# ultralytics/yolov3

Measured on NVIDIA H100. Metric: images/sec @640 bs32 YOLOv3, higher is better.
Workload: dtype bf16

## Files before the change

### include/yolov3_b200.h

```cpp
#ifndef YOLOV3_B200_H
#define YOLOV3_B200_H

#include <stddef.h>
#include <stdint.h>

#ifdef __cplusplus
extern "C" {
#endif

#define Y3_OK 0
#define Y3_ERR_BAD_ARG (-1)
#define Y3_ERR_CUDA (-2)
#define Y3_ERR_UNSUPPORTED (-3)

#define Y3_ACT_NONE 0
#define Y3_ACT_SILU 1

typedef void* y3_stream_t;

int y3_version(void);
int y3_last_error(char* buf, size_t n);
int y3_device_check(void);
int64_t y3_abi_sizeof(int32_t which);
int y3_set_pdl(int32_t on);

typedef struct y3_conv_desc {
  int32_t n, h, w;
  int32_t c_in, c_out;
  int32_t ksize, stride;
  int32_t act;
  const void* in;
  int32_t in_ld, in_coff;
  const void* weight;
  const float* bias;
  void* out;
  int32_t out_ld, out_coff;
  const void* res;
  int32_t res_ld, res_coff;
  int32_t upsample;
  float* out_f32;
  int32_t out_f32_ld;
  int32_t* err;
  int32_t weight_layout;
  int32_t in_fmt;
  int32_t out_fmt;
  const float* dq;
  float res_scale;
  float out_inv_scale;
} y3_conv_desc;
#define Y3_FMT_BF16 0
#define Y3_FMT_E4M3 1
int y3_conv_bn_act_fwd(const y3_conv_desc* d, y3_stream_t stream);
int y3_conv_dgrad_s2(const y3_conv_desc* d, y3_stream_t stream);
#define Y3_W_TAPS 0
#define Y3_W_XPAIR 1
int y3_conv_weight_layout(const y3_conv_desc* d);
typedef struct y3_conv_plan_info {
  int32_t block_n, block_k, halo, resident_weights, xpair;
  int32_t m_tiles, n_tiles, k_blocks, grid;
} y3_conv_plan_info;
int y3_conv_plan(const y3_conv_desc* d, y3_conv_plan_info* out);
int y3_conv_cout_pad(int32_t c_out);

#define Y3_IN_F32 0
#define Y3_IN_U8 1
typedef struct y3_first_desc {
  const void* in;
  int32_t in_dtype;
  float in_div;
  int32_t n, h, w;
  const float* weight;
  const float* bias;
  int32_t c_out;
  void* out;
  int32_t out_ld, out_coff;
} y3_first_desc;
int y3_conv_first_fwd(const y3_first_desc* d, y3_stream_t stream);

typedef struct y3_pool_desc {
  const void* in;
  int32_t in_ld, in_coff;
  void* out;
  int32_t out_ld, out_coff;
  int32_t n, h, w, c;
  int32_t ho, wo;
  int32_t k, stride, off, oob_zero;
  int32_t fmt;
} y3_pool_desc;
int y3_maxpool_fwd(const y3_pool_desc* d, y3_stream_t stream);
int y3_maxpool_train_fwd(const y3_pool_desc* d, uint8_t* idx, y3_stream_t stream);
int y3_maxpool_bwd(const y3_pool_desc* d, const uint8_t* idx, int32_t accumulate, y3_stream_t stream);

int y3_amax_nhwc(const void* x, int32_t fmt, int32_t ld, int32_t coff, int32_t n, int32_t h, int32_t w, int32_t c,
                 float* amax, y3_stream_t stream);

int y3_nchw_to_padded_nhwc(const float* src, int32_t n, int32_t c, int32_t h, int32_t w, void* dst, int32_t dst_ld,
                           int32_t dst_coff, y3_stream_t stream);
int y3_padded_nhwc_to_nchw(const void* src, int32_t src_ld, int32_t src_coff, int32_t n, int32_t c, int32_t h,
                           int32_t w, float* dst, y3_stream_t stream);

#define Y3_MAX_LEVELS 5
#define Y3_MAX_ANCHORS 6
typedef struct y3_detect_level {
  const float* raw;
  const float* head;
  int32_t head_ld;
  float* raw_out;
  int32_t ny, nx;
  float stride;
  float anchor_w[Y3_MAX_ANCHORS];
  float anchor_h[Y3_MAX_ANCHORS];
} y3_detect_level;
// ... 257 lines not shown
```

### yolov3_b200/_lib.py

```python
from __future__ import annotations

import ctypes as C
from pathlib import Path

_LIB_PATH = Path(__file__).resolve().parent / "libyolov3_b200.so"
_lib = None


class Y3Error(RuntimeError):
    pass


class ConvDesc(C.Structure):

    _fields_ = [
        ("n", C.c_int32), ("h", C.c_int32), ("w", C.c_int32),
        ("c_in", C.c_int32), ("c_out", C.c_int32),
        ("ksize", C.c_int32), ("stride", C.c_int32),
        ("act", C.c_int32),
        ("in_", C.c_void_p), ("in_ld", C.c_int32), ("in_coff", C.c_int32),
        ("weight", C.c_void_p),
        ("bias", C.c_void_p),
        ("out", C.c_void_p), ("out_ld", C.c_int32), ("out_coff", C.c_int32),
        ("res", C.c_void_p), ("res_ld", C.c_int32), ("res_coff", C.c_int32),
        ("upsample", C.c_int32),
        ("out_f32", C.c_void_p), ("out_f32_ld", C.c_int32),
        ("err", C.c_void_p),
        ("weight_layout", C.c_int32),
        ("in_fmt", C.c_int32), ("out_fmt", C.c_int32),
        ("dq", C.c_void_p), ("res_scale", C.c_float), ("out_inv_scale", C.c_float),
    ]


class ConvPlanInfo(C.Structure):

    _fields_ = [(k, C.c_int32) for k in ("block_n", "block_k", "halo", "resident_weights", "xpair", "m_tiles", "n_tiles",
                                         "k_blocks", "grid")]


W_TAPS, W_XPAIR = 0, 1
FMT_BF16, FMT_E4M3 = 0, 1
MAX_LEVELS, MAX_ANCHORS = 5, 6


class DetectLevel(C.Structure):

    _fields_ = [("raw", C.c_void_p), ("head", C.c_void_p), ("head_ld", C.c_int32), ("raw_out", C.c_void_p),
                ("ny", C.c_int32), ("nx", C.c_int32), ("stride", C.c_float),
                ("anchor_w", C.c_float * MAX_ANCHORS), ("anchor_h", C.c_float * MAX_ANCHORS)]


class FirstDesc(C.Structure):

    _fields_ = [("in_", C.c_void_p), ("in_dtype", C.c_int32), ("in_div", C.c_float),
                ("n", C.c_int32), ("h", C.c_int32), ("w", C.c_int32),
                ("weight", C.c_void_p), ("bias", C.c_void_p), ("c_out", C.c_int32),
                ("out", C.c_void_p), ("out_ld", C.c_int32), ("out_coff", C.c_int32)]


class PoolDesc(C.Structure):

    _fields_ = [("in_", C.c_void_p), ("in_ld", C.c_int32), ("in_coff", C.c_int32),
                ("out", C.c_void_p), ("out_ld", C.c_int32), ("out_coff", C.c_int32),
                ("n", C.c_int32), ("h", C.c_int32), ("w", C.c_int32), ("c", C.c_int32),
                ("ho", C.c_int32), ("wo", C.c_int32),
                ("k", C.c_int32), ("stride", C.c_int32), ("off", C.c_int32), ("oob_zero", C.c_int32),
                ("fmt", C.c_int32)]


class DecodeDesc(C.Structure):

    _fields_ = [("levels", DetectLevel * MAX_LEVELS), ("nl", C.c_int32), ("bs", C.c_int32), ("na", C.c_int32),
                ("no", C.c_int32), ("z", C.c_void_p)]


OP_CONV_FIRST, OP_CONV, OP_MAXPOOL, OP_DECODE, OP_AMAX = 1, 2, 3, 4, 5
IN_F32, IN_U8 = 0, 1


class AmaxDesc(C.Structure):

    _fields_ = [("x", C.c_void_p), ("fmt", C.c_int32), ("ld", C.c_int32), ("coff", C.c_int32),
                ("n", C.c_int32), ("h", C.c_int32), ("w", C.c_int32), ("c", C.c_int32), ("amax", C.c_void_p)]


class Op(C.Structure):

    _fields_ = [("kind", C.c_int32), ("conv", ConvDesc), ("first", FirstDesc), ("pool", PoolDesc),
                ("decode", DecodeDesc), ("amax", AmaxDesc)]

# ... 244 lines not shown
```

### yolov3_b200/csrc/y3_conv_tc.cu

```cuda
#include <cuda_bf16.h>

#include <type_traits>

#include "y3_common.cuh"
#include "y3_internal.h"

namespace y3 {

namespace {

constexpr int kBlockM = 128;
constexpr int kThreads = 320;
constexpr int kProducerWarp = 8;
constexpr int kStoreWarp = 9;
constexpr int kSmemBudget = 221 * 1024;

template <int BLOCK_N, int BLOCK_K, bool HALO, int STAGE_ES = 2, bool STAGE_DQ = false>
struct Cfg {
  static constexpr uint32_t kARows = HALO ? kBlockM + 2 : kBlockM;
  static constexpr uint32_t kATxBytes = kARows * BLOCK_K * 2;
  static constexpr uint32_t kABytes = (kATxBytes + 1023u) / 1024u * 1024u;
  static constexpr uint32_t kTaps = HALO ? 3 : 1;
  static constexpr uint32_t kBBytes = BLOCK_N * BLOCK_K * 2;
  static constexpr uint32_t kStageBytes = kABytes + kTaps * kBBytes;
  static constexpr int kMaxStages = 8;
  static constexpr uint32_t kBarBytes = 256;
  static constexpr uint32_t kRowBytes = BLOCK_N * (STAGE_ES > 0 ? STAGE_ES : 2);
  static constexpr uint32_t kTileBytes = kBlockM * kRowBytes;
  static constexpr uint32_t kBoxBytes = kRowBytes < 128 ? kRowBytes : 128;
  static constexpr uint32_t kBoxes = kRowBytes / kBoxBytes;
  static constexpr int kBufs = STAGE_ES == 0 ? 0 : (kTileBytes > 32 * 1024 ? 1 : 2);
  static constexpr bool kSBias = BLOCK_N == 256 && kBufs > 0;
  static constexpr uint32_t kBiasBytes = kSBias ? BLOCK_N * 4 * (STAGE_DQ ? 2 : 1) : 0;
  static constexpr uint32_t kTileReserve = 1024 - kBarBytes + kBufs * (kTileBytes + kBiasBytes);
  __host__ __device__ static constexpr int ring_stages(uint32_t reserve) {
    const int s = int(kSmemBudget - reserve) / int(kStageBytes);
    return s > kMaxStages ? kMaxStages : s;
  }
  __host__ __device__ static constexpr uint32_t bres_bytes(int steps) { return (uint32_t(steps) * kBBytes + 1023u) / 1024u * 1024u; }
  __host__ __device__ static constexpr int bres_stages(int steps, uint32_t reserve) {
    const int s = (int(kSmemBudget - reserve) - int(bres_bytes(steps))) / int(kABytes);
    return s > kMaxStages ? kMaxStages : s;
  }
  static constexpr uint32_t kSwizzleBytes = BLOCK_K * 2;
  static constexpr uint32_t kSbo = 8 * kSwizzleBytes;
  __host__ __device__ static constexpr uint32_t bar_offset(int stages, bool bres, int b_steps) {
    return uint32_t(stages) * kABytes + (bres ? bres_bytes(b_steps) : uint32_t(stages) * kTaps * kBBytes);
  }
  __host__ __device__ static constexpr uint32_t smem_end(int stages, bool bres, int b_steps, uint32_t reserve) {
    return bar_offset(stages, bres, b_steps) + kBarBytes + reserve;
  }
  static constexpr size_t kSmemBytes = size_t(kSmemBudget) + 1024  + kBarBytes;
  static_assert(ring_stages(kTileReserve) >= 2, "pipeline needs at least two stages");
  static_assert(!HALO || BLOCK_K >= 32, "halo reuse: rows of 64 or 128 bytes");
};

__device__ __forceinline__ float bias_act(float a, float b, bool silu) {
  if (!silu) return a + b;
  const float h = fmaf(a, 0.5f, b);
  float t;
  asm("tanh.approx.f32 %0, %1;" : "=f"(t) : "f"(h));
  return fmaf(h, t, h);
}

__device__ __forceinline__ float bias_act_dq(float a, float s, float b, bool silu) {
  const float h = fmaf(a, s, b);
  if (!silu) return h;
  float t;
  asm("tanh.approx.f32 %0, %1;" : "=f"(t) : "f"(h));
  return fmaf(h, t, h);
}

__device__ __forceinline__ uint32_t fast_div(uint32_t n, uint32_t mul, uint32_t shr) {
  const uint32_t t = __umulhi(n, mul);
  return (t + ((n - t) >> (shr ? 1 : 0))) >> (shr ? shr - 1 : 0);
}

struct RowOut {
  __nv_bfloat16* out;
  float* f32;
  const __nv_bfloat16* res;
};

template <int ES, typename T>
__device__ __forceinline__ T* elem_ptr(T* p, long long off) {
  if (ES == 2) return p + off;
  return reinterpret_cast<T*>(reinterpret_cast<uintptr_t>(p) + off * ES);
}

template <int ES = 2>
__device__ __forceinline__ RowOut row_out(const ConvTcArgs& p, int mt, int n0, int m) {
  RowOut o{nullptr, nullptr, nullptr};
  bool valid;
  int img, oy, ox;
  if (p.mode == 0) {
    const int row = mt * kBlockM + m;
    const int plane = p.hp * p.wp;
    img = static_cast<int>(fast_div(static_cast<uint32_t>(row), p.plane_mul, p.plane_shr));
    const int rem = row - img * plane;
    const int yp = static_cast<int>(fast_div(static_cast<uint32_t>(rem), p.wp_mul, p.wp_shr)), xp = rem - yp * p.wp;
    valid = row < p.rows_total && yp >= 1 && yp <= p.hp - 2 && xp >= 1 && xp <= p.wp - 2;
    oy = yp - 1;
    ox = xp - 1;
  } else {
    const int per_img = p.tiles_w * p.tiles_h;
    img = mt / per_img;
    const int t = mt - img * per_img;
    const int ty = m / p.tw, tx = m - ty * p.tw;
    oy = (t / p.tiles_w) * p.th + ty;
    ox = (t % p.tiles_w) * p.tw + tx;
    valid = ty < p.th && oy < p.ho && ox < p.wo;
  }
  if (!valid) return o;
  const int oh = p.mode == 0 ? p.hp - 2 : p.ho;
  const int ow = p.mode == 0 ? p.wp - 2 : p.wo;
  long long conv_row = (static_cast<long long>(img) * (oh + 2) + oy + 1) * (ow + 2) + ox + 1;
  if (p.phase)
    conv_row = (static_cast<long long>(img) * (2 * oh + 2) + 2 * oy + p.ph_a + 1) * (2 * ow + 2) + 2 * ox + p.ph_b + 1;
  if (p.res) o.res = elem_ptr<ES>(p.res, conv_row * p.res_ld + p.res_coff + n0);
  if (p.out_f32) {
    o.f32 = p.out_f32 + ((static_cast<long long>(img) * oh + oy) * ow + ox) * p.out_f32_ld + n0;
  } else if (p.upsample) {
    const long long r00 = (static_cast<long long>(img) * (2 * oh + 2) + 2 * oy + 1) * (2 * ow + 2) + 2 * ox + 1;
    o.out = elem_ptr<ES>(p.out, r00 * p.out_ld + p.out_coff + n0);
  } else {
    o.out = elem_ptr<ES>(p.out, conv_row * p.out_ld + p.out_coff + n0);
  }
  return o;
}

template <int BLOCK_N, int BLOCK_K, bool HALO, int IN_FMT = Y3_FMT_BF16, int OUT_FMT = Y3_FMT_BF16>
__global__ void __launch_bounds__(kThreads, 1)
conv_tc_kernel(const __grid_constant__ CUtensorMap map_a, const __grid_constant__ CUtensorMap map_b,
               const __grid_constant__ CUtensorMap map_out, const __grid_constant__ CUtensorMap map_res, const ConvTcArgs p) {
  constexpr bool kInE4m3 = IN_FMT == Y3_FMT_E4M3, kOutE4m3 = OUT_FMT == Y3_FMT_E4M3;
  using C = Cfg<BLOCK_N, BLOCK_K, HALO, kOutE4m3 ? 1 : (kInE4m3 ? 0 : 2), kInE4m3 && kOutE4m3>;
  constexpr int kOes = kOutE4m3 ? 1 : 2;
  constexpr int kKch = kInE4m3 ? 2 * BLOCK_K : BLOCK_K;
  using Mma = std::conditional_t<kInE4m3, WgmmaE4m3<BLOCK_N>, Wgmma<BLOCK_N>>;
  const int STAGES = p.stages;
  const bool bres = p.bres != 0;
  constexpr uint32_t kBStage = C::kTaps * C::kBBytes;
  const int b_steps = p.taps * p.kblocks;

  extern __shared__ uint8_t smem_raw[];
  const uint32_t raw_addr = smem_u32(smem_raw);
  uint8_t* smem = smem_raw + ((1024u - (raw_addr & 1023u)) & 1023u);
  uint8_t* smem_a = smem;
  uint8_t* smem_b = smem + STAGES * C::kABytes;
  uint64_t* full_bar = reinterpret_cast<uint64_t*>(smem_b + (bres ? C::bres_bytes(b_steps) : uint32_t(STAGES) * kBStage));
  uint64_t* empty_bar = full_bar + C::kMaxStages;
  uint64_t* bres_bar = empty_bar + C::kMaxStages;
  uint64_t* staged_bar = bres_bar + 1;
  uint64_t* done_bar = bres_bar + 3;
  uint8_t* otile = reinterpret_cast<uint8_t*>(full_bar) + 1024;
  const bool tile_out = C::kBufs > 0 && p.tile_tma != 0;
  constexpr int kBufs = C::kBufs > 0 ? C::kBufs : 1;

  const int warp = threadIdx.x >> 5;
  const int lane = threadIdx.x & 31;

  if (threadIdx.x == 0) {
    tma_prefetch_desc(&map_a);
    tma_prefetch_desc(&map_b);
    if (tile_out) {
      tma_prefetch_desc(&map_out);
      if (p.res) tma_prefetch_desc(&map_res);
    }
    for (int i = 0; i < STAGES; ++i) {
      mbar_init(&full_bar[i], 1);
      mbar_init(&empty_bar[i], 8);
    }
    mbar_init(bres_bar, 1);
    for (int b = 0; b < 2; ++b) {
      mbar_init(&staged_bar[b], 1);
      mbar_init(&done_bar[b], 8);
    }
    fence_mbar_init();
  }
  __syncthreads();
  pdl_wait();
  pdl_trigger();

  const int total_tiles = p.m_tiles * p.n_tiles;
  const int k_iters = HALO ? 3 * p.kblocks : p.taps * p.kblocks;

  if (warp == kProducerWarp) {
    uint32_t stage = 0, phase = 0;
    if (bres && int(blockIdx.x) < total_tiles && elect_one()) {
      mbar_expect_tx(bres_bar, uint32_t(b_steps) * C::kBBytes);
      for (int st = 0; st < b_steps; ++st) {
        const int kb = st / p.taps, tap = st - kb * p.taps;
        tma_load_2d(smem_b + st * C::kBBytes, &map_b, bres_bar, (p.custom_taps ? p.tap_wcol[tap] : tap) * p.cin + kb * kKch, 0);
      }
    }
    __syncwarp();
    const int n_tiles = p.n_tiles, wp = p.wp, cin = p.cin, a_coff = p.a_coff, a_ld = p.a_ld;
    const int taps_it = HALO ? 3 : p.taps;
    const bool xpair = p.xpair != 0, nine = p.taps == 9, custom = p.custom_taps != 0;
    const int taps_w = xpair ? 2 : 3;
    const uint32_t stage_tx = p.a_tx_bytes + (bres ? 0u : kBStage);
    auto run = [&](auto mode_tag) {
      constexpr int MODE = decltype(mode_tag)::value;
      for (int tile = blockIdx.x; tile < total_tiles; tile += gridDim.x) {
        const int nt = tile % n_tiles;
        const int mt = tile / n_tiles;
        const int n0 = nt * BLOCK_N;
        int row0 = 0, img = 0, oh0 = 0, ow0 = 0;
        if (MODE == 0) {
          row0 = mt * kBlockM;
        } else {
          const int per_img = p.tiles_w * p.tiles_h;
          img = mt / per_img;
          const int t = mt - img * per_img;
          oh0 = (t / p.tiles_w) * p.th;
          ow0 = (t % p.tiles_w) * p.tw;
        }
        int kb = 0, tap = 0, r = 0, s = 0;
        for (int it = 0; it < k_iters; ++it) {
          mbar_wait(&empty_bar[stage], phase ^ 1u, p.err, 1);
          if (elect_one()) {
            uint8_t* a_dst = smem_a + stage * C::kABytes;
            uint8_t* b_dst = smem_b + stage * kBStage;
            const int kcol = kb * kKch;
            const int shift = HALO ? (tap - 1) * wp - 1 : (custom ? p.tap_shift[tap] : (nine ? (r - 1) * wp + (s - 1) : 0));
            const int c0 = xpair ? a_coff : (s & 1) * a_ld + a_coff + kcol;
            const int c1 = xpair ? s : (s >> 1);
            const int bcol = (HALO ? tap * 3 : (custom ? p.tap_wcol[tap] : tap)) * cin + kcol;
            mbar_expect_tx(&full_bar[stage], stage_tx);
            if (MODE == 0)
              tma_load_2d(a_dst, &map_a, &full_bar[stage], a_coff + kcol, row0 + shift);
            else
              tma_load_5d(a_dst, &map_a, &full_bar[stage], c0, ow0 + c1, r & 1, oh0 + (r >> 1), img);
            if (!bres) {
#pragma unroll
              for (uint32_t t = 0; t < C::kTaps; ++t)
                tma_load_2d(b_dst + t * C::kBBytes, &map_b, &full_bar[stage], bcol + int(t) * cin, n0);
            }
          }
          __syncwarp();
          if (++stage == uint32_t(STAGES)) {
            stage = 0;
            phase ^= 1u;
          }
          if (++s == taps_w) {
            s = 0;
            ++r;
          }
          if (++tap == taps_it) {
            tap = 0;
            r = 0;
            s = 0;
            ++kb;
          }
        }
      }
    };
    if (p.mode == 0)
      run(std::integral_constant<int, 0>{});
    else
      run(std::integral_constant<int, 1>{});
  } else if (warp == kStoreWarp) {
    if (tile_out) {
      if (lane != 0) return;
      const uint32_t res_tx = uint32_t(p.mode == 0 ? kBlockM : p.tw * p.th) * C::kRowBytes;
      constexpr int kBoxCh = C::kBoxBytes / kOes;
      auto move = [&](int tile, int b, bool load) {
        const int mt = tile / p.n_tiles, n0 = (tile % p.n_tiles) * BLOCK_N;
        int c1 = mt * kBlockM, c2 = 0, c3 = 0;
        if (p.mode != 0) {
          const int per_img = p.tiles_w * p.tiles_h;
          c3 = mt / per_img;
          const int t = mt - c3 * per_img;
          c1 = (t % p.tiles_w) * p.tw;
          c2 = (t / p.tiles_w) * p.th;
        }
#pragma unroll
        for (uint32_t k = 0; k < C::kBoxes; ++k) {
          uint8_t* s = otile + b * C::kTileBytes + k * kBlockM * C::kBoxBytes;
          const int c0 = (load ? p.res_coff : p.out_coff) + n0 + int(k) * kBoxCh;
          if (load) {
            if (p.mode == 0) tma_load_2d(s, &map_res, &staged_bar[b], c0, c1);
            else tma_load_4d(s, &map_res, &staged_bar[b], c0, c1, c2, c3);
          } else {
            if (p.mode == 0) tma_store_2d(&map_out, s, c0, c1);
            else tma_store_4d(&map_out, s, c0, c1, c2, c3);
          }
        }
      };
      auto stage = [&](int tile, int b) {
        const int n0 = (tile % p.n_tiles) * BLOCK_N;
        const uint32_t bias_tx = C::kSBias ? uint32_t(min(BLOCK_N, p.cout - n0)) * 4u : 0u;
        const uint32_t tx = (p.res ? res_tx : 0u) + bias_tx * (kInE4m3 ? 2u : 1u);
        if (tx == 0) {
          mbar_arrive(&staged_bar[b]);
          return;
        }
        mbar_expect_tx(&staged_bar[b], tx);
        if (p.res) move(tile, b, true);
        if constexpr (C::kSBias) {
          uint8_t* sb = otile + C::kBufs * C::kTileBytes + b * C::kBiasBytes;
          bulk_load(sb, p.bias + n0, bias_tx, &staged_bar[b]);
          if (kInE4m3) bulk_load(sb + BLOCK_N * 4, p.dq + n0, bias_tx, &staged_bar[b]);
        }
      };
      const int step = int(gridDim.x);
#pragma unroll
      for (int i = 0; i < kBufs; ++i)
        if (int(blockIdx.x) + i * step < total_tiles) stage(blockIdx.x + i * step, i);
      for (int tile = blockIdx.x, i = 0; tile < total_tiles; tile += step, ++i) {
        const int b = i % kBufs;
        mbar_wait(&done_bar[b], uint32_t(i / kBufs) & 1u, p.err, 9);
        move(tile, b, false);
        bulk_commit_group();
        if (tile + kBufs * step < total_tiles) {
          bulk_wait_read_all();
          stage(tile + kBufs * step, b);
        }
      }
      bulk_wait_all();
    }
  } else {
    const int wg = warp >> 2;
    const int m0 = wg * 64 + (warp & 3) * 16 + (lane >> 2);
    const int cq = 2 * (lane & 3);
    constexpr uint32_t kDescHi = wgmma_desc_hi(C::kSbo, C::kSwizzleBytes);
    const uint32_t a_base = smem_u32(smem_a) + uint32_t(wg) * 64u * C::kSwizzleBytes;
    const uint32_t b_base = smem_u32(smem_b);
    uint32_t stage = 0, phase = 0;
    if (bres && int(blockIdx.x) < total_tiles) mbar_wait(bres_bar, 0, p.err, 6);
    for (int tile = blockIdx.x; tile < total_tiles; tile += gridDim.x) {
      float acc[BLOCK_N / 2];
      uint32_t prev = 0;
      for (int it = 0; it < k_iters; ++it) {
        mbar_wait(&full_bar[stage], phase, p.err, 3);
        const uint32_t a_st = a_base + stage * C::kABytes;
        const uint32_t b_st = b_base + (bres ? uint32_t(it) : stage) * kBStage;
        wgmma_fence();
#pragma unroll
        for (uint32_t t = 0; t < C::kTaps; ++t) {
#pragma unroll
          for (int k = 0; k < BLOCK_K / 16; ++k) {
            const uint64_t adesc = wgmma_desc(kDescHi, a_st + t * C::kSwizzleBytes + k * 32);
            const uint64_t bdesc = wgmma_desc(kDescHi, b_st + t * C::kBBytes + k * 32);
            Mma::template mma<0, 0>(acc, adesc, bdesc, (it != 0 || t != 0 || k != 0) ? 1u : 0u);
          }
        }
        wgmma_commit();
        wgmma_wait<1>();
        if (it > 0 && lane == 0) mbar_arrive(&empty_bar[prev]);
        prev = stage;
        if (++stage == uint32_t(STAGES)) {
          stage = 0;
          phase ^= 1u;
        }
      }
      wgmma_wait<0>();
      wgmma_fence_regs(acc);
      if (lane == 0) mbar_arrive(&empty_bar[prev]);

      const bool silu = p.act == Y3_ACT_SILU;
      const float bscale = silu ? 0.5f : 1.0f;
      if (tile_out) {
        const int ti = (tile - int(blockIdx.x)) / int(gridDim.x);
        const int b = ti % kBufs;
        mbar_wait(&staged_bar[b], uint32_t(ti / kBufs) & 1u, p.err, 10);
        const int n0 = (tile % p.n_tiles) * BLOCK_N;
        const bool has_res = p.res != nullptr;
        const uint32_t sw = ((uint32_t(m0) * C::kBoxBytes >> 7) & (C::kBoxBytes / 16 - 1)) << 4;
        const uint32_t row_s = ((smem_u32(otile) + uint32_t(m0) * C::kBoxBytes + cq * kOes) ^ sw) + b * C::kTileBytes;
        const uint32_t bias_s = smem_u32(otile) + C::kBufs * C::kTileBytes + b * C::kBiasBytes + cq * 4;
        bool valid[2] = {true, true};
        if (p.mode == 0) {
#pragma unroll
          for (int h = 0; h < 2; ++h) {
            const int row = (tile / p.n_tiles) * kBlockM + m0 + 8 * h;
            const int img = static_cast<int>(fast_div(static_cast<uint32_t>(row), p.plane_mul, p.plane_shr));
            const int rem = row - img * (p.hp * p.wp);
            const int yp = static_cast<int>(fast_div(static_cast<uint32_t>(rem), p.wp_mul, p.wp_shr)), xp = rem - yp * p.wp;
            valid[h] = yp >= 1 && yp <= p.hp - 2 && xp >= 1 && xp <= p.wp - 2;
          }
        }
#pragma unroll
        for (int j = 0; j < BLOCK_N / 8; ++j) {
          const int c = 8 * j + cq;
          float2 bv, qv;
          if constexpr (C::kSBias) {
            bv = lds_f32x2(bias_s + 32 * j);
            qv = kInE4m3 ? lds_f32x2(bias_s + 4 * BLOCK_N + 32 * j) : bv;
          } else {
            const bool in = n0 + c < p.cout;
            bv = in ? __ldg(reinterpret_cast<const float2*>(p.bias + n0 + c)) : make_float2(0.f, 0.f);
            qv = bv;
            if (kInE4m3) qv = in ? __ldg(reinterpret_cast<const float2*>(p.dq + n0 + c)) : make_float2(0.f, 0.f);
          }
          const uint32_t xb = uint32_t(8 * j * kOes);
          const uint32_t region = xb / C::kBoxBytes * (kBlockM * C::kBoxBytes), xin = xb % C::kBoxBytes;
#pragma unroll
          for (int h = 0; h < 2; ++h) {
            const uint32_t pp = (row_s ^ xin) + region + 8 * h * C::kBoxBytes;
            float x0, x1;
            if (kInE4m3) {
              x0 = bias_act_dq(acc[4 * j + 2 * h], bscale * qv.x, bscale * bv.x, silu);
              x1 = bias_act_dq(acc[4 * j + 2 * h + 1], bscale * qv.y, bscale * bv.y, silu);
            } else {
              x0 = bias_act(acc[4 * j + 2 * h], bscale * bv.x, silu);
              x1 = bias_act(acc[4 * j + 2 * h + 1], bscale * bv.y, silu);
            }
            if constexpr (kOutE4m3) {
              if (has_res) {
                const float2 f = unpack_e4m3x2(lds16(pp));
                x0 = fmaf(p.res_scale, f.x, x0);
// ... 28 lines not shown
            uint32_t r[kChunk];
#pragma unroll
            for (int jj = 0; jj < kChunk; ++jj) {
              const int c = 8 * (j0 + jj) + cq;
              const bool in = p.out_f32 || n0 + c < p.cout;
              b[jj] = in ? __ldg(reinterpret_cast<const float2*>(p.bias + n0 + c)) : make_float2(0.f, 0.f);
              if (kInE4m3) q[jj] = in ? __ldg(reinterpret_cast<const float2*>(p.dq + n0 + c)) : make_float2(0.f, 0.f);
              if (kOutE4m3)
                r[jj] = (in && ro.res) ? __ldcg(reinterpret_cast<const unsigned short*>(elem_ptr<1>(ro.res, c))) : 0u;
              else
                r[jj] = (in && ro.res) ? __ldcg(reinterpret_cast<const unsigned int*>(ro.res + c)) : 0u;
            }
#pragma unroll
            for (int jj = 0; jj < kChunk; ++jj) {
              const int c = 8 * (j0 + jj) + cq;
              if (!p.out_f32 && n0 + c >= p.cout) continue;
              float x0, x1;
              if (kInE4m3) {
                x0 = bias_act_dq(acc[4 * (j0 + jj) + 2 * h], bscale * q[jj].x, bscale * b[jj].x, silu);
                x1 = bias_act_dq(acc[4 * (j0 + jj) + 2 * h + 1], bscale * q[jj].y, bscale * b[jj].y, silu);
              } else {
                x0 = bias_act(acc[4 * (j0 + jj) + 2 * h], bscale * b[jj].x, silu);
                x1 = bias_act(acc[4 * (j0 + jj) + 2 * h + 1], bscale * b[jj].y, silu);
              }
              if (ro.f32) {
                *reinterpret_cast<float2*>(ro.f32 + c) = make_float2(x0, x1);
              } else if (kOutE4m3) {
                if (ro.res) {
                  const float2 f = unpack_e4m3x2(static_cast<uint16_t>(r[jj]));
                  x0 = fmaf(p.res_scale, f.x, x0);
                  x1 = fmaf(p.res_scale, f.y, x1);
                }
                const uint16_t v = pack_e4m3x2(x0 * p.out_inv_scale, x1 * p.out_inv_scale);
                for (int rep = 0; rep < reps; ++rep)
                  *reinterpret_cast<uint16_t*>(elem_ptr<1>(ro.out, (rep >> 1) * up_row_stride + (rep & 1) * p.out_ld + c)) = v;
              } else {
                if (ro.res) {
                  const float2 f = unpack_bf16x2(r[jj]);
                  x0 += f.x;
                  x1 += f.y;
                }
                const uint32_t v = pack_bf16x2(x0, x1);
                for (int rep = 0; rep < reps; ++rep)
                  *reinterpret_cast<uint32_t*>(ro.out + (rep >> 1) * up_row_stride + (rep & 1) * p.out_ld + c) = v;
              }
            }
          }
        }
      }
    }
  }
}

template <int BLOCK_N, int BLOCK_K, bool HALO = false, int IN_FMT = Y3_FMT_BF16, int OUT_FMT = Y3_FMT_BF16>
int launch_cfg(const ConvTcPlan& plan, cudaStream_t stream) {
  constexpr bool kInE4m3 = IN_FMT == Y3_FMT_E4M3, kOutE4m3 = OUT_FMT == Y3_FMT_E4M3;
  using C = Cfg<BLOCK_N, BLOCK_K, HALO, kOutE4m3 ? 1 : (kInE4m3 ? 0 : 2), kInE4m3 && kOutE4m3>;
  auto kern = conv_tc_kernel<BLOCK_N, BLOCK_K, HALO, IN_FMT, OUT_FMT>;
  static bool attr_set = false;
  if (!attr_set) {
    Y3_CHECK_CUDA(cudaFuncSetAttribute(kern, cudaFuncAttributeMaxDynamicSharedMemorySize, int(C::kSmemBytes)));
    attr_set = true;
  }
  ConvTcArgs args = plan.args;
  const uint32_t reserve = (C::kBufs > 0 && args.tile_tma != 0) ? C::kTileReserve : 0u;
  const int b_steps = args.taps * args.kblocks;
  args.bres = plan.bres;
  args.stages = plan.bres ? C::bres_stages(b_steps, reserve) : C::ring_stages(reserve);
  if (args.bres && args.stages < 3) {
    args.bres = 0;
    args.stages = C::ring_stages(reserve);
  }
  if (args.stages < 2 || args.stages > C::kMaxStages ||
      C::smem_end(args.stages, args.bres != 0, b_steps, reserve) + 1024u > C::kSmemBytes)
    return set_error(Y3_ERR_BAD_ARG, "conv_tc: %d ring stages (resident weights %d, output tiles %u bytes) do not fit %zu bytes of shared memory (N=%d K=%d)",
                     args.stages, args.bres, reserve, C::kSmemBytes, BLOCK_N, BLOCK_K);
  Y3_CHECK_CUDA(launch_pdl(kern, dim3(plan.grid), dim3(kThreads), C::kSmemBytes, stream, plan.map_a, plan.map_b,
                           plan.map_out, plan.map_res, args));
  return Y3_OK;
}

int pick_block_n(int cout) { return cout <= 32 ? 32 : (cout <= 64 ? 64 : (cout <= 128 ? 128 : 256)); }

template <int IN_FMT, int OUT_FMT>
int launch_fmt(const ConvTcPlan& plan, cudaStream_t stream) {
#define Y3_DISPATCH_K(BN)                                                        \
  switch (plan.block_k) {                                                        \
    case 64: return launch_cfg<BN, 64, false, IN_FMT, OUT_FMT>(plan, stream);    \
    case 32: return launch_cfg<BN, 32, false, IN_FMT, OUT_FMT>(plan, stream);    \
    case 16: return launch_cfg<BN, 16, false, IN_FMT, OUT_FMT>(plan, stream);    \
  }                                                                              \
  break;
  constexpr bool kHalo = !(IN_FMT == Y3_FMT_E4M3 && OUT_FMT == Y3_FMT_BF16);
  if (plan.halo) {
    if constexpr (kHalo) {
      if (plan.block_k == 64) {
        if (plan.block_n == 128) return launch_cfg<128, 64, true, IN_FMT, OUT_FMT>(plan, stream);
        if (plan.block_n == 64) return launch_cfg<64, 64, true, IN_FMT, OUT_FMT>(plan, stream);
        if (plan.block_n == 32) return launch_cfg<32, 64, true, IN_FMT, OUT_FMT>(plan, stream);
      } else if (plan.block_k == 32) {
        if (plan.block_n == 64) return launch_cfg<64, 32, true, IN_FMT, OUT_FMT>(plan, stream);
        if (plan.block_n == 32) return launch_cfg<32, 32, true, IN_FMT, OUT_FMT>(plan, stream);
      }
    }
    return set_error(Y3_ERR_BAD_ARG, "conv_tc: no halo kernel for tile N=%d K=%d (formats %d -> %d)", plan.block_n,
                     plan.block_k, IN_FMT, OUT_FMT);
  }
  switch (plan.block_n) {
    case 32: Y3_DISPATCH_K(32)
    case 64: Y3_DISPATCH_K(64)
    case 128: Y3_DISPATCH_K(128)
    case 256: Y3_DISPATCH_K(256)
  }
#undef Y3_DISPATCH_K
  return set_error(Y3_ERR_BAD_ARG, "conv_tc: no kernel for tile N=%d K=%d", plan.block_n, plan.block_k);
}

}

int conv_tc_launch(const ConvTcPlan& plan, cudaStream_t stream) {
  if (plan.in_fmt == Y3_FMT_BF16 && plan.out_fmt == Y3_FMT_BF16) return launch_fmt<Y3_FMT_BF16, Y3_FMT_BF16>(plan, stream);
  if (plan.in_fmt == Y3_FMT_BF16 && plan.out_fmt == Y3_FMT_E4M3) return launch_fmt<Y3_FMT_BF16, Y3_FMT_E4M3>(plan, stream);
  if (plan.in_fmt == Y3_FMT_E4M3 && plan.out_fmt == Y3_FMT_E4M3) return launch_fmt<Y3_FMT_E4M3, Y3_FMT_E4M3>(plan, stream);
  if (plan.in_fmt == Y3_FMT_E4M3 && plan.out_fmt == Y3_FMT_BF16) return launch_fmt<Y3_FMT_E4M3, Y3_FMT_BF16>(plan, stream);
  return set_error(Y3_ERR_BAD_ARG, "conv_tc: formats %d -> %d", plan.in_fmt, plan.out_fmt);
}

static void fast_div_for(uint32_t d, uint32_t* mul, uint32_t* shr) {
  if (d <= 1) {
    *mul = 0;
    *shr = 0;
    return;
  }
  uint32_t l = 0;
  while ((1ull << l) < d) ++l;
  *mul = static_cast<uint32_t>(((1ull << 32) * ((1ull << l) - d)) / d + 1);
  *shr = l;
}

static bool conv_prefers_xpair(const y3_conv_desc& d) {
  return d.in_fmt == Y3_FMT_BF16 && d.ksize == 3 && d.stride == 2 && (d.c_in == 32 || d.c_in == 16) && d.in_ld == d.c_in && d.in_coff == 0;
}

int conv_tc_prepare(const y3_conv_desc& d, ConvTcPlan* plan, bool select_only, const ConvTcExtra* extra) {
  Y3_REQUIRE(d.n > 0 && d.h > 0 && d.w > 0, "conv: empty shape");
  Y3_REQUIRE((d.ksize == 1 && d.stride == 1) || (d.ksize == 3 && (d.stride == 1 || d.stride == 2)),
// ... 49 lines not shown
  const int kch = bk * 2 / es;
  const int cout_pad = (d.c_out + bn - 1) / bn * bn;
  const int taps = extra ? extra->ntaps : (xpair ? 6 : d.ksize * d.ksize);
  const int hp = d.h + 2, wp = d.w + 2;
  if (extra) Y3_REQUIRE(d.stride == 1 && !xpair && !head && !d.upsample && extra->ntaps >= 1 && extra->ntaps <= 4, "conv: bad custom tap list");

  ConvTcArgs& a = plan->args;
  a = ConvTcArgs{};
  plan->in_fmt = d.in_fmt;
  plan->out_fmt = out8 ? Y3_FMT_E4M3 : Y3_FMT_BF16;
  plan->block_n = bn;
  plan->block_k = bk;
  a.taps = taps;
  a.kblocks = gemm_cin / kch;
  a.cin = gemm_cin;
  a.xpair = xpair ? 1 : 0;
  a.a_coff = d.in_coff;
  a.a_ld = d.in_ld;
  a.n_tiles = cout_pad / bn;
  a.bias = d.bias;
  a.cout = d.c_out;
  a.act = d.act;
  a.out = static_cast<__nv_bfloat16*>(d.out);
  a.out_ld = d.out_ld;
  a.out_coff = d.out_coff;
  a.upsample = d.upsample;
  a.res = static_cast<const __nv_bfloat16*>(d.res);
  a.res_ld = d.res_ld;
  a.res_coff = d.res_coff;
  a.out_f32 = d.out_f32;
  a.out_f32_ld = d.out_f32_ld;
  a.err = d.err;
  a.dq = in8 ? d.dq : nullptr;
  a.res_scale = d.res_scale;
  a.out_inv_scale = d.out_inv_scale;
  if (head) {
    a.out = nullptr;
    Y3_REQUIRE(d.out_f32_ld >= (d.c_out + pick_block_n(d.c_out) - 1) / pick_block_n(d.c_out) * pick_block_n(d.c_out),
               "conv: out_f32_ld must cover the padded c_out");
  }

  int rc;
  if (d.stride == 1) {
    a.mode = 0;
    a.hp = hp;
    a.wp = wp;
    fast_div_for(static_cast<uint32_t>(hp) * wp, &a.plane_mul, &a.plane_shr);
    fast_div_for(static_cast<uint32_t>(wp), &a.wp_mul, &a.wp_shr);
    const long long rows = static_cast<long long>(d.n) * hp * wp;
    Y3_REQUIRE(rows < (1ll << 31) - 4096, "conv: too many pixels");
    a.rows_total = static_cast<int>(rows);
    a.m_tiles = static_cast<int>((rows + kBlockM - 1) / kBlockM);
    plan->halo = (!extra && taps == 9 && ((bk == 64 && bn <= 128) || (bk == 32 && bn <= 64))) ? 1 : 0;
    if (extra) {
      a.custom_taps = 1;
      for (int t = 0; t < extra->ntaps; ++t) {
        a.tap_shift[t] = extra->dr[t] * wp + extra->ds[t];
        a.tap_wcol[t] = extra->wcol[t];
      }
      a.phase = extra->phase;
      a.ph_a = extra->ph_a;
      a.ph_b = extra->ph_b;
    }
    const uint32_t a_rows = plan->halo ? kBlockM + 2 : kBlockM;
    a.a_tx_bytes = a_rows * bk * 2;
    const uint64_t dims[2] = {static_cast<uint64_t>(d.in_ld), static_cast<uint64_t>(rows)};
    const uint64_t strides[2] = {0, static_cast<uint64_t>(d.in_ld) * es};
    const uint32_t box[2] = {static_cast<uint32_t>(kch), a_rows};
    rc = select_only ? Y3_OK : encode_tensor_map(&plan->map_a, d.in_fmt, d.in, 2, dims, strides, box, bk * 2);
    if (rc) return rc;
  } else {
    plan->halo = 0;
    a.mode = 1;
    a.ho = d.h / 2;
    a.wo = d.w / 2;
    int best_tw = 1, best_th = 1;
    long long best_tiles = -1;
    for (int tw = 1; tw <= 128 && tw <= 256; ++tw) {
      const int th = 128 / tw;
      if (th < 1) break;
      const int thc = th > a.ho ? a.ho : th;
      const long long tiles = static_cast<long long>((a.wo + tw - 1) / tw) * ((a.ho + thc - 1) / thc);
      if (best_tiles < 0 || tiles < best_tiles || (tiles == best_tiles && tw > best_tw)) {
        best_tiles = tiles;
        best_tw = tw;
        best_th = thc;
      }
    }
    a.tw = best_tw;
    a.th = best_th;
    a.tiles_w = (a.wo + a.tw - 1) / a.tw;
    a.tiles_h = (a.ho + a.th - 1) / a.th;
    a.m_tiles = d.n * a.tiles_w * a.tiles_h;
    a.a_tx_bytes = static_cast<uint32_t>(a.tw) * a.th * bk * 2;
    const uint64_t ld = static_cast<uint64_t>(d.in_ld);
    const uint64_t dims[5] = {2 * ld, static_cast<uint64_t>(wp / 2), 2, static_cast<uint64_t>(hp / 2),
                              static_cast<uint64_t>(d.n)};
    const uint64_t strides[5] = {0, 2 * ld * es, static_cast<uint64_t>(wp) * ld * es, 2ull * wp * ld * es,
                                 static_cast<uint64_t>(hp) * wp * ld * es};
    const uint32_t box[5] = {static_cast<uint32_t>(kch), static_cast<uint32_t>(a.tw), 1, static_cast<uint32_t>(a.th), 1};
    rc = select_only ? Y3_OK : encode_tensor_map(&plan->map_a, d.in_fmt, d.in, 5, dims, strides, box, bk * 2);
    if (rc) return rc;
  }
  {
    const uint64_t ktot = static_cast<uint64_t>(extra ? d.ksize * d.ksize : taps) * gemm_cin;
    const uint64_t dims[2] = {ktot, static_cast<uint64_t>(cout_pad)};
    const uint64_t strides[2] = {0, ktot * es};
    const uint32_t box[2] = {static_cast<uint32_t>(kch), static_cast<uint32_t>(bn)};
    rc = select_only ? Y3_OK : encode_tensor_map(&plan->map_b, d.in_fmt, d.weight, 2, dims, strides, box, bk * 2);
    if (rc) return rc;
  }
  plan->map_out = CUtensorMap{};
  plan->map_res = CUtensorMap{};
  a.tile_tma = (!head && !d.upsample && !(extra && extra->phase)) ? 1 : 0;
  if (a.tile_tma && !select_only) {
    const int oes = out8 ? 1 : 2;
    const int box_bytes = bn * oes < 128 ? bn * oes : 128;
    const uint32_t box_ch = static_cast<uint32_t>(box_bytes / oes);
    auto encode_out = [&](CUtensorMap* m, const void* base, int ld, int coff) {
      const uint64_t pitch = static_cast<uint64_t>(ld) * oes;
      if (a.mode == 0) {
        const uint64_t dims[2] = {static_cast<uint64_t>(coff + d.c_out), static_cast<uint64_t>(a.rows_total)};
        const uint64_t strides[2] = {0, pitch};
        const uint32_t box[2] = {box_ch, kBlockM};
        return encode_tensor_map(m, plan->out_fmt, base, 2, dims, strides, box, box_bytes);
      }
      const uint64_t wpo = static_cast<uint64_t>(a.wo) + 2, hpo = static_cast<uint64_t>(a.ho) + 2;
      const void* interior = static_cast<const uint8_t*>(base) + (wpo + 1) * pitch;
      const uint64_t dims[4] = {static_cast<uint64_t>(coff + d.c_out), static_cast<uint64_t>(a.wo),
                                static_cast<uint64_t>(a.ho), static_cast<uint64_t>(d.n)};
      const uint64_t strides[4] = {0, pitch, wpo * pitch, hpo * wpo * pitch};
      const uint32_t box[4] = {box_ch, static_cast<uint32_t>(a.tw), static_cast<uint32_t>(a.th), 1};
      return encode_tensor_map(m, plan->out_fmt, interior, 4, dims, strides, box, box_bytes);
    };
    rc = encode_out(&plan->map_out, d.out, d.out_ld, d.out_coff);
    if (rc) return rc;
    if (d.res) {
      rc = encode_out(&plan->map_res, d.res, d.res_ld, d.res_coff);
      if (rc) return rc;
    }
  }
  {
    const long long b_bytes = static_cast<long long>(taps) * a.kblocks * bn * bk * 2;
    plan->bres = (a.n_tiles == 1 && b_bytes <= 96 * 1024) ? 1 : 0;
  }
  const int sms = num_sms();
  const long long total = static_cast<long long>(a.m_tiles) * a.n_tiles;
  plan->grid = static_cast<int>(total < sms ? total : sms);
  return Y3_OK;
}

}

extern "C" int y3_conv_plan(const y3_conv_desc* d, y3_conv_plan_info* out) {
  if (!d || !out) return y3::set_error(Y3_ERR_BAD_ARG, "conv_plan: null argument");
  y3::ConvTcPlan plan;
  int rc = y3::conv_tc_prepare(*d, &plan, true);
  if (rc) return rc;
  out->block_n = plan.block_n;
  out->block_k = plan.block_k;
  out->halo = plan.halo;
  out->resident_weights = plan.bres;
  out->xpair = plan.args.xpair;
  out->m_tiles = plan.args.m_tiles;
  out->n_tiles = plan.args.n_tiles;
  out->k_blocks = plan.args.kblocks;
  out->grid = plan.grid;
  return Y3_OK;
}

extern "C" int y3_conv_weight_layout(const y3_conv_desc* d) {
  if (!d) return y3::set_error(Y3_ERR_BAD_ARG, "conv: null descriptor");
  return y3::conv_prefers_xpair(*d) ? Y3_W_XPAIR : Y3_W_TAPS;
}

extern "C" int y3_conv_cout_pad(int32_t c_out) {
  const int bn = y3::pick_block_n(c_out);
  return (c_out + bn - 1) / bn * bn;
}

extern "C" int y3_conv_dgrad_s2(const y3_conv_desc* d, y3_stream_t stream) {
  if (!d) return y3::set_error(Y3_ERR_BAD_ARG, "conv: null descriptor");
  Y3_REQUIRE(d->ksize == 3 && d->stride == 1 && !d->upsample && !d->out_f32 && d->weight_layout == Y3_W_TAPS,
             "dgrad_s2: describe the 3x3 transposed conv on dy's own grid (stride 1 in the descriptor), bf16 output");
  for (int a = 0; a < 2; ++a)
    for (int b = 0; b < 2; ++b) {
      y3::ConvTcExtra ex{};
      ex.phase = 1;
      ex.ph_a = a;
      ex.ph_b = b;
      const int rs[2][2] = {{1, -1}, {0, 2}};
      for (int ri = 0; ri < 2; ++ri) {
        const int r = rs[a][ri];
        if (r < 0) continue;
        for (int si = 0; si < 2; ++si) {
          const int s = rs[b][si];
          if (s < 0) continue;
          const int t = ex.ntaps++;
          ex.dr[t] = (a == 1 && r == 0) ? 1 : 0;
          ex.ds[t] = (b == 1 && s == 0) ? 1 : 0;
          ex.wcol[t] = (2 - r) * 3 + (2 - s);
        }
      }
      y3::ConvTcPlan plan;
      int rc = y3::conv_tc_prepare(*d, &plan, false, &ex);
      if (rc) return rc;
      rc = y3::conv_tc_launch(plan, static_cast<cudaStream_t>(stream));
      if (rc) return rc;
    }
  return Y3_OK;
}

extern "C" int y3_conv_bn_act_fwd(const y3_conv_desc* d, y3_stream_t stream) {
  if (!d) return y3::set_error(Y3_ERR_BAD_ARG, "conv: null descriptor");
  y3::ConvTcPlan plan;
  int rc = y3::conv_tc_prepare(*d, &plan);
  if (rc) return rc;
  return y3::conv_tc_launch(plan, static_cast<cudaStream_t>(stream));
}
```

### yolov3_b200/csrc/y3_internal.h

```cpp
#pragma once

#include <cuda.h>
#include <cuda_bf16.h>
#include <cuda_runtime.h>
#include <stdint.h>

#include <string>

#include "../../include/yolov3_b200.h"

namespace y3 {

int set_error(int code, const char* fmt, ...);
#define Y3_CHECK_CUDA(expr)                                                                            \
  do {                                                                                                 \
    cudaError_t _e = (expr);                                                                           \
    if (_e != cudaSuccess)                                                                             \
      return ::y3::set_error(Y3_ERR_CUDA, "%s failed: %s (%s:%d)", #expr, cudaGetErrorString(_e), __FILE__, __LINE__); \
  } while (0)
#define Y3_REQUIRE(cond, ...)                                       \
  do {                                                              \
    if (!(cond)) return ::y3::set_error(Y3_ERR_BAD_ARG, __VA_ARGS__); \
  } while (0)

int encode_tensor_map(CUtensorMap* out, int fmt, const void* base, int rank, const uint64_t* dims, const uint64_t* strides,
                      const uint32_t* box, int swizzle_bytes);
inline int encode_tensor_map_bf16(CUtensorMap* out, const void* base, int rank, const uint64_t* dims, const uint64_t* strides,
                                  const uint32_t* box, int swizzle_bytes) {
  return encode_tensor_map(out, Y3_FMT_BF16, base, rank, dims, strides, box, swizzle_bytes);
}

int num_sms();
int pdl_enabled();
void pdl_set(int on);

struct ConvTcArgs {
  int mode;
  int taps, kblocks, cin;
  int a_coff, a_ld;
  uint32_t a_tx_bytes;
  int xpair;
  int stages;
  int bres;
  int m_tiles, n_tiles;
  int hp, wp, rows_total;
  uint32_t plane_mul, plane_shr, wp_mul, wp_shr;
  int tw, th, tiles_w, tiles_h, ho, wo;
  const float* bias;
  int cout, act;
  __nv_bfloat16* out;
  int out_ld, out_coff, upsample;
  const __nv_bfloat16* res;
  int res_ld, res_coff;
  float* out_f32;
  int out_f32_ld;
  int* err;
  int custom_taps;
  int tap_shift[4], tap_wcol[4];
  int phase, ph_a, ph_b;
  const float* dq;
  float res_scale, out_inv_scale;
  int tile_tma;
};

struct ConvTcExtra {
  int ntaps;
  int dr[4], ds[4];
  int wcol[4];
  int phase, ph_a, ph_b;
};

struct ConvTcPlan {
  CUtensorMap map_a, map_b;
  CUtensorMap map_out, map_res;
  int in_fmt, out_fmt;
  int halo;
  int bres;
  ConvTcArgs args;
  int block_n, block_k;
  int grid;
};
int conv_tc_prepare(const y3_conv_desc& d, ConvTcPlan* plan, bool select_only = false, const ConvTcExtra* extra = nullptr);
int conv_tc_launch(const ConvTcPlan& plan, cudaStream_t stream);
int pool_launch(const y3_pool_desc& d, cudaStream_t stream);
int amax_launch(const y3_amax_desc& d, cudaStream_t stream);
int wgrad_tc(const y3_wgrad_desc& d, cudaStream_t stream);
int pool_train_fwd(const y3_pool_desc& d, uint8_t* idx, cudaStream_t stream);
int pool_bwd(const y3_pool_desc& d, const uint8_t* idx, int accumulate, cudaStream_t stream);

}
```

Before: 2641.

## Add A-row reuse ring for N=256 stride-1 3x3 conv kernels

Adds an AROW kernel variant for 3x3 stride-1 convs with 256 output channels. It loads one halo-extended input row block (128+2 rows) per kernel row and reuses it across the three horizontal taps by shifting the shared-memory descriptor. Weights stream through their own per-tap ring. This cuts A-operand TMA traffic and shared-memory footprint, leaving room for more B stages, at the cost of a second barrier ring, finer-grained synchronization, and disabling resident weights for these layers.

```diff
diff --git a/include/yolov3_b200.h b/include/yolov3_b200.h
--- a/include/yolov3_b200.h
+++ b/include/yolov3_b200.h
@@ -58,6 +58,7 @@
 typedef struct y3_conv_plan_info {
   int32_t block_n, block_k, halo, resident_weights, xpair;
   int32_t m_tiles, n_tiles, k_blocks, grid;
+  int32_t a_row_ring;
 } y3_conv_plan_info;
 int y3_conv_plan(const y3_conv_desc* d, y3_conv_plan_info* out);
 int y3_conv_cout_pad(int32_t c_out);
diff --git a/yolov3_b200/_lib.py b/yolov3_b200/_lib.py
--- a/yolov3_b200/_lib.py
+++ b/yolov3_b200/_lib.py
@@ -35,7 +35,7 @@
 class ConvPlanInfo(C.Structure):
 
     _fields_ = [(k, C.c_int32) for k in ("block_n", "block_k", "halo", "resident_weights", "xpair", "m_tiles", "n_tiles",
-                                         "k_blocks", "grid")]
+                                         "k_blocks", "grid", "a_row_ring")]
 
 
 W_TAPS, W_XPAIR = 0, 1
diff --git a/yolov3_b200/csrc/y3_conv_tc.cu b/yolov3_b200/csrc/y3_conv_tc.cu
--- a/yolov3_b200/csrc/y3_conv_tc.cu
+++ b/yolov3_b200/csrc/y3_conv_tc.cu
@@ -38,17 +38,24 @@
     return s > kMaxStages ? kMaxStages : s;
   }
   __host__ __device__ static constexpr uint32_t bres_bytes(int steps) { return (uint32_t(steps) * kBBytes + 1023u) / 1024u * 1024u; }
+  static constexpr uint32_t kARowBytes = ((kBlockM + 2) * BLOCK_K * 2 + 1023u) / 1024u * 1024u;
+  static constexpr int kARowSlots = 2;
+  __host__ __device__ static constexpr int arow_stages(uint32_t reserve) {
+    const int s = (int(kSmemBudget - reserve) - kARowSlots * int(kARowBytes)) / int(kBBytes);
+    return s > kMaxStages ? kMaxStages : s;
+  }
   __host__ __device__ static constexpr int bres_stages(int steps, uint32_t reserve) {
     const int s = (int(kSmemBudget - reserve) - int(bres_bytes(steps))) / int(kABytes);
     return s > kMaxStages ? kMaxStages : s;
   }
   static constexpr uint32_t kSwizzleBytes = BLOCK_K * 2;
   static constexpr uint32_t kSbo = 8 * kSwizzleBytes;
-  __host__ __device__ static constexpr uint32_t bar_offset(int stages, bool bres, int b_steps) {
-    return uint32_t(stages) * kABytes + (bres ? bres_bytes(b_steps) : uint32_t(stages) * kTaps * kBBytes);
-  }
-  __host__ __device__ static constexpr uint32_t smem_end(int stages, bool bres, int b_steps, uint32_t reserve) {
-    return bar_offset(stages, bres, b_steps) + kBarBytes + reserve;
+  __host__ __device__ static constexpr uint32_t bar_offset(int stages, bool bres, int b_steps, bool arow = false) {
+    return (arow ? kARowSlots * kARowBytes : uint32_t(stages) * kABytes) +
+           (bres ? bres_bytes(b_steps) : uint32_t(stages) * kTaps * kBBytes);
+  }
+  __host__ __device__ static constexpr uint32_t smem_end(int stages, bool bres, int b_steps, uint32_t reserve, bool arow = false) {
+    return bar_offset(stages, bres, b_steps, arow) + kBarBytes + reserve;
   }
   static constexpr size_t kSmemBytes = size_t(kSmemBudget) + 1024  + kBarBytes;
   static_assert(ring_stages(kTileReserve) >= 2, "pipeline needs at least two stages");
@@ -129,7 +136,7 @@
   return o;
 }
 
-template <int BLOCK_N, int BLOCK_K, bool HALO, int IN_FMT = Y3_FMT_BF16, int OUT_FMT = Y3_FMT_BF16>
+template <int BLOCK_N, int BLOCK_K, bool HALO, int IN_FMT = Y3_FMT_BF16, int OUT_FMT = Y3_FMT_BF16, bool AROW = false>
 __global__ void __launch_bounds__(kThreads, 1)
 conv_tc_kernel(const __grid_constant__ CUtensorMap map_a, const __grid_constant__ CUtensorMap map_b,
                const __grid_constant__ CUtensorMap map_out, const __grid_constant__ CUtensorMap map_res, const ConvTcArgs p) {
@@ -138,6 +145,7 @@
   constexpr int kOes = kOutE4m3 ? 1 : 2;
   constexpr int kKch = kInE4m3 ? 2 * BLOCK_K : BLOCK_K;
   using Mma = std::conditional_t<kInE4m3, WgmmaE4m3<BLOCK_N>, Wgmma<BLOCK_N>>;
+  static_assert(!AROW || (!HALO && BLOCK_N == 256), "A-row mode: the N = 256 stride-1 3x3 launches");
   const int STAGES = p.stages;
   const bool bres = p.bres != 0;
   constexpr uint32_t kBStage = C::kTaps * C::kBBytes;
@@ -147,12 +155,14 @@
   const uint32_t raw_addr = smem_u32(smem_raw);
   uint8_t* smem = smem_raw + ((1024u - (raw_addr & 1023u)) & 1023u);
   uint8_t* smem_a = smem;
-  uint8_t* smem_b = smem + STAGES * C::kABytes;
+  uint8_t* smem_b = smem + (AROW ? C::kARowSlots * C::kARowBytes : STAGES * C::kABytes);
   uint64_t* full_bar = reinterpret_cast<uint64_t*>(smem_b + (bres ? C::bres_bytes(b_steps) : uint32_t(STAGES) * kBStage));
   uint64_t* empty_bar = full_bar + C::kMaxStages;
   uint64_t* bres_bar = empty_bar + C::kMaxStages;
   uint64_t* staged_bar = bres_bar + 1;
   uint64_t* done_bar = bres_bar + 3;
+  uint64_t* arow_full = bres_bar + 5;
+  uint64_t* arow_empty = bres_bar + 7;
   uint8_t* otile = reinterpret_cast<uint8_t*>(full_bar) + 1024;
   const bool tile_out = C::kBufs > 0 && p.tile_tma != 0;
   constexpr int kBufs = C::kBufs > 0 ? C::kBufs : 1;
@@ -175,6 +185,12 @@
     for (int b = 0; b < 2; ++b) {
       mbar_init(&staged_bar[b], 1);
       mbar_init(&done_bar[b], 8);
+    }
+    if (AROW) {
+      for (int a = 0; a < C::kARowSlots; ++a) {
+        mbar_init(&arow_full[a], 1);
+        mbar_init(&arow_empty[a], 8);
+      }
     }
     fence_mbar_init();
   }
@@ -256,10 +272,43 @@
         }
       }
     };
-    if (p.mode == 0)
+    if constexpr (AROW) {
+      uint32_t aslot = 0, aphase = 0;
+      for (int tile = blockIdx.x; tile < total_tiles; tile += gridDim.x) {
+        const int row0 = (tile / n_tiles) * kBlockM, n0 = (tile % n_tiles) * BLOCK_N;
+        for (int kb = 0; kb < p.kblocks; ++kb) {
+          const int kcol = kb * kKch;
+          for (int r = 0; r < 3; ++r) {
+            mbar_wait(&arow_empty[aslot], aphase ^ 1u, p.err, 11);
+            if (elect_one()) {
+              mbar_expect_tx(&arow_full[aslot], p.a_tx_bytes);
+              tma_load_2d(smem_a + aslot * C::kARowBytes, &map_a, &arow_full[aslot], a_coff + kcol, row0 + (r - 1) * wp - 1);
+            }
+            __syncwarp();
+            if (++aslot == uint32_t(C::kARowSlots)) {
+              aslot = 0;
+              aphase ^= 1u;
+            }
+            for (int t = 3 * r; t < 3 * r + 3; ++t) {
+              mbar_wait(&empty_bar[stage], phase ^ 1u, p.err, 1);
+              if (elect_one()) {
+                mbar_expect_tx(&full_bar[stage], C::kBBytes);
+                tma_load_2d(smem_b + stage * C::kBBytes, &map_b, &full_bar[stage], t * cin + kcol, n0);
+              }
+              __syncwarp();
+              if (++stage == uint32_t(STAGES)) {
+                stage = 0;
+                phase ^= 1u;
+              }
+            }
+          }
+        }
+      }
+    } else if (p.mode == 0) {
       run(std::integral_constant<int, 0>{});
-    else
+    } else {
       run(std::integral_constant<int, 1>{});
+    }
   } else if (warp == kStoreWarp) {
     if (tile_out) {
       if (lane != 0) return;
@@ -328,36 +377,81 @@
     const uint32_t a_base = smem_u32(smem_a) + uint32_t(wg) * 64u * C::kSwizzleBytes;
     const uint32_t b_base = smem_u32(smem_b);
     uint32_t stage = 0, phase = 0;
+    uint32_t aslot = 0, aphase = 0;
     if (bres && int(blockIdx.x) < total_tiles) mbar_wait(bres_bar, 0, p.err, 6);
     for (int tile = blockIdx.x; tile < total_tiles; tile += gridDim.x) {
       float acc[BLOCK_N / 2];
       uint32_t prev = 0;
-      for (int it = 0; it < k_iters; ++it) {
-        mbar_wait(&full_bar[stage], phase, p.err, 3);
-        const uint32_t a_st = a_base + stage * C::kABytes;
-        const uint32_t b_st = b_base + (bres ? uint32_t(it) : stage) * kBStage;
-        wgmma_fence();
-#pragma unroll
-        for (uint32_t t = 0; t < C::kTaps; ++t) {
-#pragma unroll
-          for (int k = 0; k < BLOCK_K / 16; ++k) {
-            const uint64_t adesc = wgmma_desc(kDescHi, a_st + t * C::kSwizzleBytes + k * 32);
-            const uint64_t bdesc = wgmma_desc(kDescHi, b_st + t * C::kBBytes + k * 32);
-            Mma::template mma<0, 0>(acc, adesc, bdesc, (it != 0 || t != 0 || k != 0) ? 1u : 0u);
-          }
-        }
-        wgmma_commit();
-        wgmma_wait<1>();
-        if (it > 0 && lane == 0) mbar_arrive(&empty_bar[prev]);
-        prev = stage;
-        if (++stage == uint32_t(STAGES)) {
-          stage = 0;
-          phase ^= 1u;
-        }
-      }
-      wgmma_wait<0>();
-      wgmma_fence_regs(acc);
-      if (lane == 0) mbar_arrive(&empty_bar[prev]);
+      if constexpr (AROW) {
+        for (int kb = 0; kb < p.kblocks; ++kb) {
+#pragma unroll 1
+          for (int r = 0; r < 3; ++r) {
+            mbar_wait(&arow_full[aslot], aphase, p.err, 12);
+            const uint32_t a_st = a_base + aslot * C::kARowBytes;
+#pragma unroll 1
+            for (int s = 0; s < 3; ++s) {
+              const bool first = (kb | r | s) == 0;
+              mbar_wait(&full_bar[stage], phase, p.err, 3);
+              const uint32_t b_st = b_base + stage * C::kBBytes;
+              wgmma_fence();
+#pragma unroll
+              for (int k = 0; k < BLOCK_K / 16; ++k) {
+                const uint64_t adesc = wgmma_desc(kDescHi, a_st + s * C::kSwizzleBytes + k * 32);
+                const uint64_t bdesc = wgmma_desc(kDescHi, b_st + k * 32);
+                Mma::template mma<0, 0>(acc, adesc, bdesc, (!first || k != 0) ? 1u : 0u);
+              }
+              wgmma_commit();
+              wgmma_wait<1>();
+              if (!first && lane == 0) {
+                mbar_arrive(&empty_bar[prev]);
+                if (s == 0) mbar_arrive(&arow_empty[aslot ^ 1u]);
+              }
+              prev = stage;
+              if (++stage == uint32_t(STAGES)) {
+                stage = 0;
+                phase ^= 1u;
+              }
+            }
+            if (++aslot == uint32_t(C::kARowSlots)) {
+              aslot = 0;
+              aphase ^= 1u;
+            }
+          }
+        }
+        wgmma_wait<0>();
+        wgmma_fence_regs(acc);
+        if (lane == 0) {
+          mbar_arrive(&empty_bar[prev]);
+          mbar_arrive(&arow_empty[aslot ^ 1u]);
+        }
+      } else {
+        for (int it = 0; it < k_iters; ++it) {
+          mbar_wait(&full_bar[stage], phase, p.err, 3);
+          const uint32_t a_st = a_base + stage * C::kABytes;
+          const uint32_t b_st = b_base + (bres ? uint32_t(it) : stage) * kBStage;
+          wgmma_fence();
+#pragma unroll
+          for (uint32_t t = 0; t < C::kTaps; ++t) {
+#pragma unroll
+            for (int k = 0; k < BLOCK_K / 16; ++k) {
+              const uint64_t adesc = wgmma_desc(kDescHi, a_st + t * C::kSwizzleBytes + k * 32);
+              const uint64_t bdesc = wgmma_desc(kDescHi, b_st + t * C::kBBytes + k * 32);
+              Mma::template mma<0, 0>(acc, adesc, bdesc, (it != 0 || t != 0 || k != 0) ? 1u : 0u);
+            }
+          }
+          wgmma_commit();
+          wgmma_wait<1>();
+          if (it > 0 && lane == 0) mbar_arrive(&empty_bar[prev]);
+          prev = stage;
+          if (++stage == uint32_t(STAGES)) {
+            stage = 0;
+            phase ^= 1u;
+          }
+        }
+        wgmma_wait<0>();
+        wgmma_fence_regs(acc);
+        if (lane == 0) mbar_arrive(&empty_bar[prev]);
+      }
 
       const bool silu = p.act == Y3_ACT_SILU;
       const float bscale = silu ? 0.5f : 1.0f;
@@ -492,11 +586,11 @@
   }
 }
 
-template <int BLOCK_N, int BLOCK_K, bool HALO = false, int IN_FMT = Y3_FMT_BF16, int OUT_FMT = Y3_FMT_BF16>
+template <int BLOCK_N, int BLOCK_K, bool HALO = false, int IN_FMT = Y3_FMT_BF16, int OUT_FMT = Y3_FMT_BF16, bool AROW = false>
 int launch_cfg(const ConvTcPlan& plan, cudaStream_t stream) {
   constexpr bool kInE4m3 = IN_FMT == Y3_FMT_E4M3, kOutE4m3 = OUT_FMT == Y3_FMT_E4M3;
   using C = Cfg<BLOCK_N, BLOCK_K, HALO, kOutE4m3 ? 1 : (kInE4m3 ? 0 : 2), kInE4m3 && kOutE4m3>;
-  auto kern = conv_tc_kernel<BLOCK_N, BLOCK_K, HALO, IN_FMT, OUT_FMT>;
+  auto kern = conv_tc_kernel<BLOCK_N, BLOCK_K, HALO, IN_FMT, OUT_FMT, AROW>;
   static bool attr_set = false;
   if (!attr_set) {
     Y3_CHECK_CUDA(cudaFuncSetAttribute(kern, cudaFuncAttributeMaxDynamicSharedMemorySize, int(C::kSmemBytes)));
@@ -505,14 +599,14 @@
   ConvTcArgs args = plan.args;
   const uint32_t reserve = (C::kBufs > 0 && args.tile_tma != 0) ? C::kTileReserve : 0u;
   const int b_steps = args.taps * args.kblocks;
-  args.bres = plan.bres;
-  args.stages = plan.bres ? C::bres_stages(b_steps, reserve) : C::ring_stages(reserve);
+  args.bres = AROW ? 0 : plan.bres;
+  args.stages = AROW ? C::arow_stages(reserve) : (plan.bres ? C::bres_stages(b_steps, reserve) : C::ring_stages(reserve));
   if (args.bres && args.stages < 3) {
     args.bres = 0;
     args.stages = C::ring_stages(reserve);
   }
   if (args.stages < 2 || args.stages > C::kMaxStages ||
-      C::smem_end(args.stages, args.bres != 0, b_steps, reserve) + 1024u > C::kSmemBytes)
+      C::smem_end(args.stages, args.bres != 0, b_steps, reserve, AROW) + 1024u > C::kSmemBytes)
     return set_error(Y3_ERR_BAD_ARG, "conv_tc: %d ring stages (resident weights %d, output tiles %u bytes) do not fit %zu bytes of shared memory (N=%d K=%d)",
                      args.stages, args.bres, reserve, C::kSmemBytes, BLOCK_N, BLOCK_K);
   Y3_CHECK_CUDA(launch_pdl(kern, dim3(plan.grid), dim3(kThreads), C::kSmemBytes, stream, plan.map_a, plan.map_b,
@@ -532,6 +626,13 @@
   }                                                                              \
   break;
   constexpr bool kHalo = !(IN_FMT == Y3_FMT_E4M3 && OUT_FMT == Y3_FMT_BF16);
+  if (plan.arow) {
+    if constexpr (kHalo) {
+      if (plan.block_n == 256 && plan.block_k == 64) return launch_cfg<256, 64, false, IN_FMT, OUT_FMT, true>(plan, stream);
+    }
+    return set_error(Y3_ERR_BAD_ARG, "conv_tc: no A-row kernel for tile N=%d K=%d (formats %d -> %d)", plan.block_n,
+                     plan.block_k, IN_FMT, OUT_FMT);
+  }
   if (plan.halo) {
     if constexpr (kHalo) {
       if (plan.block_k == 64) {
@@ -687,6 +788,7 @@
     a.rows_total = static_cast<int>(rows);
     a.m_tiles = static_cast<int>((rows + kBlockM - 1) / kBlockM);
     plan->halo = (!extra && taps == 9 && ((bk == 64 && bn <= 128) || (bk == 32 && bn <= 64))) ? 1 : 0;
+    plan->arow = (!extra && taps == 9 && bk == 64 && bn == 256 && cout_pad == 256) ? 1 : 0;
     if (extra) {
       a.custom_taps = 1;
       for (int t = 0; t < extra->ntaps; ++t) {
@@ -697,7 +799,7 @@
       a.ph_a = extra->ph_a;
       a.ph_b = extra->ph_b;
     }
-    const uint32_t a_rows = plan->halo ? kBlockM + 2 : kBlockM;
+    const uint32_t a_rows = (plan->halo || plan->arow) ? kBlockM + 2 : kBlockM;
     a.a_tx_bytes = a_rows * bk * 2;
     const uint64_t dims[2] = {static_cast<uint64_t>(d.in_ld), static_cast<uint64_t>(rows)};
     const uint64_t strides[2] = {0, static_cast<uint64_t>(d.in_ld) * es};
@@ -706,6 +808,7 @@
     if (rc) return rc;
   } else {
     plan->halo = 0;
+    plan->arow = 0;
     a.mode = 1;
     a.ho = d.h / 2;
     a.wo = d.w / 2;
@@ -777,7 +880,7 @@
   }
   {
     const long long b_bytes = static_cast<long long>(taps) * a.kblocks * bn * bk * 2;
-    plan->bres = (a.n_tiles == 1 && b_bytes <= 96 * 1024) ? 1 : 0;
+    plan->bres = (!plan->arow && a.n_tiles == 1 && b_bytes <= 96 * 1024) ? 1 : 0;
   }
   const int sms = num_sms();
   const long long total = static_cast<long long>(a.m_tiles) * a.n_tiles;
@@ -801,6 +904,7 @@
   out->n_tiles = plan.args.n_tiles;
   out->k_blocks = plan.args.kblocks;
   out->grid = plan.grid;
+  out->a_row_ring = plan.arow;
   return Y3_OK;
 }
 
diff --git a/yolov3_b200/csrc/y3_internal.h b/yolov3_b200/csrc/y3_internal.h
--- a/yolov3_b200/csrc/y3_internal.h
+++ b/yolov3_b200/csrc/y3_internal.h
@@ -76,6 +76,7 @@
   int in_fmt, out_fmt;
   int halo;
   int bres;
+  int arow;
   ConvTcArgs args;
   int block_n, block_k;
   int grid;
```

Measured after the change: 2651 (median of 6 runs). No clear change (+0.4%).
